# Plonky3/Plonky3-recursion

Measured on AMD Instinct MI355X. Metric: prove_next_layer ms + Poseidon2 perms/s, KoalaBear 2^20-row circuit, 1/8 GPU, lower is better.
Workload: dtype u32 Montgomery (31-bit prime field, degree-4 extension); Poseidon2 hashing as exact integers in f64; 1 GPU; prove_next_layer (verifier-circuit run on the device + prove_all_tables) of the synthetic koala-bear 2^20-row recursion layer: tables const/public/alu/poseidon2/recompose, FRI blowup 4, arity<=4, 54 queries, 15-bit PoW; circuit inputs + NextLayerPrepCache resident in HBM; field=koala-bear, log_height=20, independent_proofs=1, proof_bytes=612900, parallelism=1 independent proofs, one per GPU, no data-path collective

## Files before the change

plonky3_recursion_amd/csrc/kernels_coop.hip.h:

```cpp
#pragma once
#include "kernels.hip.h"

namespace p3r {

template <int CTRL>
__device__ __forceinline__ uint32_t dpp(uint32_t v) {
  return (uint32_t)__builtin_amdgcn_update_dpp(0, (int)v, CTRL, 0xF, 0xF, false);
}
constexpr int DPP_QUAD_NEXT1 = 0x39;
constexpr int DPP_QUAD_NEXT2 = 0x4E;
constexpr int DPP_QUAD_NEXT3 = 0x93;
constexpr int DPP_ROW_ROR1 = 0x121, DPP_ROW_ROR2 = 0x122, DPP_ROW_ROR4 = 0x124, DPP_ROW_ROR8 = 0x128;

template <class F>
__device__ __forceinline__ F coop_external(F x) {
  F b = F::raw(dpp<DPP_QUAD_NEXT1>(x.v)), c = F::raw(dpp<DPP_QUAD_NEXT2>(x.v)), d = F::raw(dpp<DPP_QUAD_NEXT3>(x.v));
  F ab = x + b;
  F y = ab.dbl() + b + (c + d);
  F t = y + F::raw(dpp<DPP_ROW_ROR4>(y.v));
  t = t + F::raw(dpp<DPP_ROW_ROR8>(t.v));
  return y + t;
}
template <class F>
__device__ __forceinline__ F coop_row_sum(F x) {
// ... 2 lines not shown
  t = t + F::raw(dpp<DPP_ROW_ROR2>(t.v));
  return t + F::raw(dpp<DPP_ROW_ROR1>(t.v));
}

constexpr int DPP_QUAD_BCAST0 = 0x00;
__device__ __forceinline__ uint32_t coop_bcast0(uint32_t x0) {
  uint32_t q = dpp<DPP_QUAD_BCAST0>(x0);
  q |= dpp<DPP_ROW_ROR4>(q);
  return q | dpp<DPP_ROW_ROR8>(q);
}

template <class PP>
struct CoopRc {
  uint32_t full[2 * P2_HALF_FULL];
  uint32_t part[PP::PARTIAL_ROUNDS];
};
template <class PP>
__device__ __forceinline__ CoopRc<PP> coop_load_rc(const uint32_t* __restrict__ rc, int elem) {
  CoopRc<PP> c;
#pragma unroll
  for (int r = 0; r < P2_HALF_FULL; ++r) c.full[r] = rc[r * P2_WIDTH + elem];
#pragma unroll
  for (int r = 0; r < PP::PARTIAL_ROUNDS; ++r) c.part[r] = rc[P2_HALF_FULL * P2_WIDTH + r];
#pragma unroll
  for (int r = 0; r < P2_HALF_FULL; ++r)
    c.full[P2_HALF_FULL + r] = rc[P2_HALF_FULL * P2_WIDTH + PP::PARTIAL_ROUNDS + r * P2_WIDTH + elem];
  return c;
}

template <class PP>
__device__ __forceinline__ Fp<PP> coop_permute(Fp<PP> s, int elem, Fp<PP> diag, const CoopRc<PP>& rc) {
  using F = Fp<PP>;
  s = coop_external(s);
#pragma unroll
  for (int r = 0; r < P2_HALF_FULL; ++r) {
    s = p2_sbox<PP>(s + F::raw(rc.full[r]));
    s = coop_external(s);
  }
#pragma unroll
  for (int r = 0; r < PP::PARTIAL_ROUNDS; ++r) {
    const F rest = coop_row_sum(elem == 0 ? F::zero() : s);
    const F sb = p2_sbox<PP>(s + F::raw(rc.part[r]));
    const F sum = rest + F::raw(coop_bcast0(elem == 0 ? sb.v : 0u));
    s = (elem == 0 ? sb : s) * diag + sum;
  }
#pragma unroll
  for (int r = 0; r < P2_HALF_FULL; ++r) {
    s = p2_sbox<PP>(s + F::raw(rc.full[P2_HALF_FULL + r]));
    s = coop_external(s);
  }
  return s;
}

template <class PP>
__global__ void __launch_bounds__(kBlock)
k_mmcs_hash_rows_strided_coop(const uint32_t* const* __restrict__ cols, int wtot, size_t h, size_t stride,
                              uint32_t* __restrict__ dig, const uint32_t* __restrict__ rc,
                              const uint32_t* __restrict__ diag) {
  using F = Fp<PP>;
  const size_t gid = (size_t)blockIdx.x * kBlock + threadIdx.x;
  const size_t row = gid >> 4;
  const int e = (int)(gid & 15);
  const bool live = row < h;
  const F d = F::raw(diag[e]);
  const CoopRc<PP> rcs = coop_load_rc<PP>(rc, e);
  F s = F::zero();
  for (int g = 0; g < wtot; g += P2_RATE) {
    if (live && e < P2_RATE && g + e < wtot) s = F::raw(cols[g + e][row * stride]);
    s = coop_permute<PP>(s, e, d, rcs);
  }
  if (live && e < P2_DIGEST) dig[(size_t)e * h + row] = s.v;
}

constexpr int kSubtreeBlock = 1024;
constexpr int kSubtreeNodes = 256;
constexpr int kSubtreeLevels = 8;
struct SubtreeArgs {
  const uint32_t* in;
  uint32_t n_in;
  uint32_t local;
  int n_levels;
  uint32_t* out[kSubtreeLevels];
  const uint32_t* inj[kSubtreeLevels];
  uint32_t* t_state;
  uint32_t* t_beta;
  uint32_t* t_cap;
  int t_dc;
};

template <class PP>
__device__ __forceinline__ void fri_transcript_step(int j, uint32_t root_word, uint32_t* __restrict__ state,
                                                    uint32_t* __restrict__ beta_out, uint32_t* __restrict__ cap_out,
                                                    const CoopRc<PP>& rc, const uint32_t* __restrict__ diag, int dc = 4) {
  using F = Fp<PP>;
  F s = j < P2_RATE ? F::raw(root_word) : F::raw(state[j]);
  if (j < P2_RATE) cap_out[j] = s.v;
  if (j == P2_RATE) s += F::from_canonical(P2_RATE);
  s = coop_permute<PP>(s, j, F::raw(diag[j]), rc);
  state[j] = s.v;
  if (j >= P2_RATE - dc && j < P2_RATE) beta_out[7 - j] = s.v;
}
template <class PP>
__global__ void __launch_bounds__(kSubtreeBlock)
k_mmcs_subtree(SubtreeArgs a, const uint32_t* __restrict__ rc, const uint32_t* __restrict__ diag) {
  using F = Fp<PP>;
  __shared__ uint32_t buf[2][P2_DIGEST * kSubtreeNodes / 2];
  const int elem = threadIdx.x & 15;
  const uint32_t group = threadIdx.x >> 4, k = elem & 7;
  const F d = F::raw(diag[elem]);
  const CoopRc<PP> rcs = coop_load_rc<PP>(rc, elem);
  uint32_t n = a.n_in < a.local ? a.n_in : a.local;
  uint32_t n_glob = a.n_in, first = blockIdx.x * n;
#pragma unroll
  for (int l = 0; l < kSubtreeLevels; ++l) {
    if (l < a.n_levels) {
      const uint32_t nn = n / 2, nn_glob = n_glob / 2, first_out = first / 2;
      const uint32_t* cur = buf[(l + 1) & 1];
      uint32_t* nxt = buf[l & 1];
      for (uint32_t node = group; node < nn; node += blockDim.x / 16) {
        const uint32_t child = 2 * node + (elem >> 3);
        F s = F::raw(l == 0 ? a.in[(size_t)k * n_glob + first + child] : cur[k * n + child]);
        s = coop_permute<PP>(s, elem, d, rcs);
        if (a.inj[l]) {
          if (elem >= P2_DIGEST) s = F::raw(a.inj[l][(size_t)k * nn_glob + first_out + node]);
          s = coop_permute<PP>(s, elem, d, rcs);
        }
        if (elem < P2_DIGEST) {
          nxt[k * nn + node] = s.v;
          a.out[l][(size_t)k * nn_glob + first_out + node] = s.v;
        }
      }
      __syncthreads();
      n = nn;
      n_glob = nn_glob;
      first = first_out;
    }
  }
  if (a.t_state && threadIdx.x < P2_WIDTH) {
    const uint32_t* root = buf[(a.n_levels - 1) & 1];
    fri_transcript_step<PP>((int)threadIdx.x, threadIdx.x < P2_RATE ? root[threadIdx.x] : 0u, a.t_state, a.t_beta,
                            a.t_cap, rcs, diag, a.t_dc ? a.t_dc : 4);
  }
}

template <class PP>
__global__ void __launch_bounds__(64)
k_fri_transcript_step(const uint32_t* __restrict__ root , uint32_t* __restrict__ state ,
                      uint32_t* __restrict__ beta_out , uint32_t* __restrict__ cap_out ,
                      const uint32_t* __restrict__ rc, const uint32_t* __restrict__ diag, int dc) {
  const int j = threadIdx.x;
  if (j >= P2_WIDTH) return;
  fri_transcript_step<PP>(j, j < P2_RATE ? root[j] : 0u, state, beta_out, cap_out, coop_load_rc<PP>(rc, j), diag, dc);
}



template <class F>
__device__ __forceinline__ F coop32_pair_sum(F t) {
  const auto r = __builtin_amdgcn_permlane16_swap(t.v, t.v, false, false);
  return F::raw(r[0]) + F::raw(r[1]);
}
template <class F>
__device__ __forceinline__ F coop32_external(F x) {
  const F b = F::raw(dpp<DPP_QUAD_NEXT1>(x.v)), c = F::raw(dpp<DPP_QUAD_NEXT2>(x.v)), d = F::raw(dpp<DPP_QUAD_NEXT3>(x.v));
  const F ab = x + b;
  const F y = ab.dbl() + b + (c + d);
  F t = y + F::raw(dpp<DPP_ROW_ROR4>(y.v));
  t = t + F::raw(dpp<DPP_ROW_ROR8>(t.v));
  return y + coop32_pair_sum(t);
}
template <class F>
__device__ __forceinline__ F coop32_sum(F x) { return coop32_pair_sum(coop_row_sum(x)); }
__device__ __forceinline__ uint32_t coop32_bcast0(uint32_t x0) {
  const uint32_t q = coop_bcast0(x0);
  const auto r = __builtin_amdgcn_permlane16_swap(q, q, false, false);
  return r[0] | r[1];
}

template <class PP>
// ... 45 lines not shown
```

plonky3_recursion_amd/csrc/kernels_stark.hip.h:

```cpp
#pragma once
#include "air_device.hip.h"
#include "kernels.hip.h"

namespace p3r {

template <int DC>
struct EW {
  uint32_t c[DC];
};
using E4 = EW<4>;
template <class PP, int DC = 4>
__host__ __device__ __forceinline__ typename Chal<PP, DC>::type e4_load(const EW<DC>& e) {
  typename Chal<PP, DC>::type r;
  for (int i = 0; i < DC; ++i) r.c[i] = Fp<PP>::raw(e.c[i]);
  return r;
}
template <class PP, int DC = 4>
__host__ __device__ __forceinline__ EW<DC> e4_store(const typename Chal<PP, DC>::type& e) {
  EW<DC> r;
  for (int i = 0; i < DC; ++i) r.c[i] = e.c[i].v;
  return r;
}

template <int DC>
// ... 350 lines not shown
#pragma unroll
    for (int i = 0; i < 4; ++i) out[i] = x[i].inv();
    return;
  }
  F t = p0123.inv();
  const F i3 = t * p012;
  t = t * nm[3].d;
  const F i2 = t * p01;
  t = t * nm[2].d;
  const F i1 = t * nm[0].d, i0 = t * nm[1].d;
  out[0] = x[0].inv_given(nm[0], i0);
  out[1] = x[1].inv_given(nm[1], i1);
  out[2] = x[2].inv_given(nm[2], i2);
  out[3] = x[3].inv_given(nm[3], i3);
}

}

#include "kernels_open.hip.h"

namespace p3r {

struct FriFoldArgs {
  const uint32_t* in;
  uint32_t* out;
  size_t rows;
  int log_rows;
  const uint32_t* beta;
  const uint32_t* roll;
  uint32_t w_inv;
  uint32_t tw_inv[4][8];
  uint32_t neg_half;
};
typedef uint32_t fri_u32x2 __attribute__((ext_vector_type(2)));
typedef uint32_t fri_u32x4 __attribute__((ext_vector_type(4)));
template <class PP, int DC, int LA, int S>
__device__ __forceinline__ void fri_fold_steps(typename Chal<PP, DC>::type* e, typename Chal<PP, DC>::type& b, Fp<PP>& ss_inv,
                                               const Fp<PP> nh, const uint32_t (&tw_inv)[4][8]) {
  using F = Fp<PP>;
  using E = typename Chal<PP, DC>::type;
  if constexpr (S < LA) {
#pragma unroll
    for (int j = 0; j < (1 << (LA - S - 1)); ++j) {
      F x0_inv = ss_inv * F::raw(tw_inv[S][j]);
      E t = b * x0_inv - E::one();
      e[j] = e[2 * j] + t * (e[2 * j + 1] - e[2 * j]) * nh;
    }
    ss_inv = ss_inv.sqr();
    b = b.sqr();
    fri_fold_steps<PP, DC, LA, S + 1>(e, b, ss_inv, nh, tw_inv);
  }
}
template <class PP, int DC, int LA>
__global__ void __launch_bounds__(kBlock) k_fri_fold(FriFoldArgs a) {
  using F = Fp<PP>;
  using E = typename Chal<PP, DC>::type;
  static_assert(LA >= 1 && LA <= 4, "folds by 2, 4, 8 or 16");
  constexpr int ARITY = 1 << LA;
  size_t r = (size_t)blockIdx.x * kBlock + threadIdx.x;
  if (r >= a.rows) return;
  const size_t n_in = a.rows << LA;
  E e[ARITY];
#pragma unroll
  for (int k = 0; k < DC; ++k) {
    const gptr<const uint32_t> row = as_global(a.in) + (size_t)k * n_in + (r << LA);
    if constexpr (LA == 1) {
      const fri_u32x2 v = *(gptr<const fri_u32x2>)row;
      e[0].c[k] = F::raw(v.x);
      e[1].c[k] = F::raw(v.y);
    } else {
#pragma unroll
      for (int q = 0; q < ARITY / 4; ++q) {
        const fri_u32x4 v = ((gptr<const fri_u32x4>)row)[q];
        e[4 * q].c[k] = F::raw(v.x);
        e[4 * q + 1].c[k] = F::raw(v.y);
        e[4 * q + 2].c[k] = F::raw(v.z);
        e[4 * q + 3].c[k] = F::raw(v.w);
      }
    }
  }
  F ss_inv = F::raw(a.w_inv).pow(bit_reverse((uint32_t)r, a.log_rows));
  E b;
#pragma unroll
  for (int k = 0; k < DC; ++k) b.c[k] = F::raw(as_global(a.beta)[k]);
  fri_fold_steps<PP, DC, LA, 0>(e, b, ss_inv, F::raw(a.neg_half), a.tw_inv);
  E res = e[0];
  if (a.roll) {
    E ro;
#pragma unroll
    for (int k = 0; k < DC; ++k) ro.c[k] = F::raw(as_global(a.roll)[(size_t)k * a.rows + r]);
    res += b * ro;
  }
#pragma unroll
  for (int k = 0; k < DC; ++k) as_global(a.out)[(size_t)k * a.rows + r] = res.c[k].v;
}

template <class PP>
__global__ void __launch_bounds__(kBlock)
k_mmcs_hash_rows_strided(const uint32_t* const* __restrict__ cols, int wtot, size_t h, size_t stride,
                         uint32_t* __restrict__ dig, const double* __restrict__ rcd) {
  size_t i = (size_t)blockIdx.x * kBlock + threadIdx.x;
  if (i >= h) return;
  double s[P2_WIDTH];
#pragma unroll
  for (int k = 0; k < P2_WIDTH; ++k) s[k] = 0.0;
  int g = 0;
  for (; g + P2_RATE <= wtot; g += P2_RATE) {
#pragma unroll
    for (int j = 0; j < P2_RATE; ++j) s[j] = p2f_load<PP>(cols[g + j][i * stride]);
    p2f_permute<PP, 0xFF00u>(s, rcd);
  }
  int rem = wtot - g;
  if (rem > 0) {
#pragma unroll
    for (int j = 0; j < P2_RATE; ++j)
      if (j < rem) s[j] = p2f_load<PP>(cols[g + j][i * stride]);
    p2f_permute<PP, 0xFFFFu>(s, rcd);
  }
#pragma unroll
  for (int k = 0; k < P2_DIGEST; ++k) dig[(size_t)k * h + i] = p2f_store<PP>(s[k]);
}

struct GrindArgs {
  uint32_t state[16];
  uint32_t pending[8];
  int n_pending;
  int bits;
  uint32_t base;
  const uint32_t* rc;
  uint32_t* result;
};
template <class PP>
__global__ void __launch_bounds__(kBlock) k_grind(GrindArgs a) {
  using F = Fp<PP>;
  uint32_t cand = a.base + blockIdx.x * kBlock + threadIdx.x;
  if (cand >= PP::P) return;
  F s[P2_WIDTH];
#pragma unroll
  for (int k = 0; k < P2_WIDTH; ++k) s[k] = F::raw(a.state[k]);
  const int n_abs = a.n_pending + 1;
#pragma unroll
  for (int k = 0; k < P2_RATE; ++k) {
    if (k < a.n_pending) s[k] = F::raw(a.pending[k]);
    else if (k == a.n_pending) s[k] = F::from_canonical(cand);
    else s[k] = F::zero();
  }
  s[P2_RATE] += F::from_canonical((uint32_t)n_abs);
// ... 29 lines not shown
```

plonky3_recursion_amd/csrc/mmcs_impl.hip.h:

```cpp

namespace {

template <class PP>
void hash_rows(p3r_ctx* ctx, const std::vector<std::vector<const p3r_dmat*>>& classes,
               const std::vector<uint32_t*>& digs) {
  std::vector<HashRowsJob> jobs;
  for (size_t c = 0; c < classes.size(); ++c) {
    std::vector<const uint32_t*> cols;
    for (const p3r_dmat* m : classes[c])
      for (size_t k = 0; k < m->w; ++k) cols.push_back(m->d + k * m->h);
    HashRowsJob j{};
    j.cols = col_table(ctx, cols);
    j.dig = digs[c];
    j.h = classes[c][0]->h;
    j.wtot = (int)cols.size();
    jobs.push_back(j);
  }
  std::stable_sort(jobs.begin(), jobs.end(),
                   [](const HashRowsJob& a, const HashRowsJob& b) { return a.wtot > b.wtot; });
  uint32_t blocks = 0;
  double perms = 0;
  for (auto& j : jobs) {
    j.block0 = blocks;
    blocks += blocks_for(j.h);
    perms += (double)j.h * ((j.wtot + P2_RATE - 1) / P2_RATE);
  }
  prof_count(ctx, "hash_rows_perms", perms);
  const auto* d_jobs =
      static_cast<const HashRowsJob*>(const_table(ctx, jobs.data(), jobs.size() * sizeof(HashRowsJob)));
  ProfScope ps(ctx, "mmcs_hash_rows");
  hipLaunchKernelGGL(k_mmcs_hash_rows<PP>, dim3(blocks), dim3(kBlock), 0, ctx->stream, d_jobs, (int)jobs.size(),
                     ctx->rcd());
  P3R_HIP(hipGetLastError());
}

inline size_t env_pow2(const char* name, size_t dflt, size_t lo, size_t hi) {
  const char* e = tuning_knob(name);
  size_t v = e ? (size_t)atol(e) : dflt;
  v = std::min(std::max(v, lo), hi);
  while (v & (v - 1)) v &= v - 1;
  return v;
}
inline size_t coop_max_nodes() {
  static const size_t v = env_pow2("P3R_COOP_MAX_NODES", 16384, 1, size_t(1) << 30);
  return v;
}
inline size_t coop_max_leaf_rows() {
  static const size_t v = env_pow2("P3R_COOP_MAX_LEAF_ROWS", 8192, 1, size_t(1) << 30);
  return v;
}
inline size_t subtree_nodes() {
  static const size_t v = env_pow2("P3R_SUBTREE_NODES", 32, 2, kSubtreeNodes);
  return v;
}
template <class PP>
void launch_compress(p3r_ctx* ctx, const uint32_t* prev, const uint32_t* inj, uint32_t* out, size_t n) {
  ProfScope ps(ctx, "mmcs_compress");
  hipLaunchKernelGGL(k_mmcs_compress<PP>, dim3(blocks_for(n)), dim3(kBlock), 0, ctx->stream, prev, inj, out, n,
                     ctx->rcd());
  P3R_HIP(hipGetLastError());
}

using InjectMap = std::map<size_t, DevBuf>;
inline const uint32_t* injected_at(const InjectMap* inject, const MmcsLevel& lv) {
  if (!lv.inject_h) return nullptr;
  if (!inject || !inject->count(lv.inject_h) || lv.inject_h != lv.logical_next)
    fail(P3R_EINVAL, "MMCS: matrix heights must be powers of two");
  return inject->at(lv.inject_h).p;
}
inline void push_layer(p3r_tree* tree, size_t n) {
  tree->layers.emplace_back(P2_DIGEST * n);
  tree->layer_n.push_back(n);
}

struct TranscriptStep {
  uint32_t *state, *beta, *cap;
  bool done = false;
  int dc = 4;
};
template <class PP>
size_t mmcs_subtree(p3r_ctx* ctx, p3r_tree* tree, size_t l, const InjectMap* inject, TranscriptStep* step) {
  const size_t n = tree->layer_n.back();
  if (n / 2 > coop_max_nodes()) return 0;
  SubtreeArgs a{};
  a.in = tree->layers.back().p;
  a.n_in = (uint32_t)n;
  const size_t local = std::min<size_t>(n, subtree_nodes());
  a.local = (uint32_t)local;
  for (size_t shrink = local; shrink > 1 && l + a.n_levels < tree->levels.size() && a.n_levels < kSubtreeLevels; shrink /= 2) {
    const MmcsLevel& lv = tree->levels[l + a.n_levels];
    push_layer(tree, lv.padded_next);
    a.out[a.n_levels] = tree->layers.back().p;
    a.inj[a.n_levels] = injected_at(inject, lv);
    ++a.n_levels;
  }
  if (step && tree->layer_n.back() == 1 && n == local) {
    a.t_state = step->state;
    a.t_beta = step->beta;
    a.t_cap = step->cap;
    a.t_dc = step->dc;
    step->done = true;
// ... 220 lines not shown
```

plonky3_recursion_amd/csrc/p3r_core.hip:

```cpp
#include "context.h"
#include "kernels.hip.h"
#include "kernels_stark.hip.h"
#include "kernels_coop.hip.h"
#include "tu_api.h"
#include "profile.h"
#include "run_schedule.h"
#include "prep_device.h"
#include "host_abi.h"

#include <sys/random.h>

#include <algorithm>
#include <cerrno>
#include <future>
#include <numeric>
#include <unordered_map>

using namespace p3r;

namespace {

thread_local std::string g_create_error;

template <class Fn>
int guard(p3r_ctx* ctx, Fn&& fn) {
  try {
    if (ctx) {
      (void)hipSetDevice(ctx->cfg.device);
      tls_pool() = ctx->pool;
      if (ctx->const_tables.size() > 4096) ctx->const_tables.clear();
    }
    fn();
    return P3R_OK;
  } catch (const Error& e) {
    if (ctx) ctx->err = e.what(); else g_create_error = e.what();
    return e.code;
  } catch (const std::exception& e) {
    if (ctx) ctx->err = e.what(); else g_create_error = e.what();
    return P3R_EINVAL;
  }
}

inline void require_w32_constants(const p3r_ctx* ctx) {
  if (ctx->w32_unacknowledged)
    fail(P3R_EINVAL, "the width-32 permutation with poseidon2_w32_rc / poseidon2_w32_diag NULL: the built-in constants are self-generated, "
                     "not upstream's - pass the caller's, or acknowledge with P3R_EXT_UNPINNED_W32_DEFAULTS");
}

#define P3R_FIELD_CALL(ctx, fn, ...)                                              \
  ((ctx)->cfg.field == P3R_FIELD_KOALA_BEAR ? fn<KoalaBearParams>(__VA_ARGS__)    \
                                            : fn<BabyBearParams>(__VA_ARGS__))

inline unsigned blocks_for(size_t n) { return (unsigned)((n + kBlock - 1) / kBlock); }

template <class PP>
std::unique_ptr<p3r_dmat> upload(p3r_ctx* ctx, const uint32_t* rowmajor, size_t h, size_t w) {
// ... 925 lines not shown
```

plonky3_recursion_amd/csrc/prove_impl.hip.h:

```cpp
#include "host_transcript.h"
#include "kernels_stark.hip.h"
#include "kernels_fri_reduce.hip.h"
#include "kernels_zk.hip.h"
#include "open_impl.hip.h"

struct p3r_prep {
  std::vector<p3r::AirParams> airs;
  std::vector<std::unique_ptr<p3r_dmat>> traces;
  std::vector<std::unique_ptr<p3r_dmat>> evals;
  std::vector<std::unique_ptr<p3r_dmat>> ldes;
  std::vector<size_t> heights;
  int zk_codewords = -1;
  const p3r_dmat* committed(size_t i) const { return evals.empty() ? traces[i].get() : evals[i].get(); }
  std::unique_ptr<p3r_tree> tree;
  std::vector<uint32_t> cap_canonical;
};

namespace {

template <class PP, int DC = 4>
EW<DC> to_e4(const typename Chal<PP, DC>::type& e) { return e4_store<PP, DC>(e); }

template <class PP, int DC = 4>
std::vector<typename Chal<PP, DC>::type> download_ef(p3r_ctx* ctx, const uint32_t* dev, size_t count) {
// ... 686 lines not shown
      FriReduceJob j{};
      j.ro = ros[kv.first].second.p;
      j.h = uint64_t(1) << kv.first;
      j.mat0 = (uint32_t)mats.size();
      j.n_mats = (uint32_t)kv.second.size();
      j.block0 = blocks;
      blocks += blocks_for(size_t(1) << kv.first);
      jobs.push_back(j);
      mats.insert(mats.end(), kv.second.begin(), kv.second.end());
    }
    const size_t b_mats = mats.size() * sizeof(FriReduceMatT<DC>), b_jobs = jobs.size() * sizeof(FriReduceJob),
                 b_vsum = vsum_jobs.size() * sizeof(FriVsumJob);
    const size_t o_jobs = (b_mats + 15) & ~size_t(15), o_vsum = (o_jobs + b_jobs + 15) & ~size_t(15);
    std::vector<unsigned char> blob(o_vsum + b_vsum);
    std::memcpy(blob.data(), mats.data(), b_mats);
    std::memcpy(blob.data() + o_jobs, jobs.data(), b_jobs);
    std::memcpy(blob.data() + o_vsum, vsum_jobs.data(), b_vsum);
    keep.emplace_back((blob.size() + 3) / 4);
    unsigned char* d_blob = reinterpret_cast<unsigned char*>(keep.back().p);
    P3R_HIP(ctx->stage.upload(ctx->stream, d_blob, blob.data(), blob.size()));
    const auto* d_mats = reinterpret_cast<const FriReduceMatT<DC>*>(d_blob);
    const auto* d_jobs = reinterpret_cast<const FriReduceJob*>(d_blob + o_jobs);
    const auto* d_vsum = reinterpret_cast<const FriVsumJob*>(d_blob + o_vsum);
    {
      ProfScope ps(ctx, "fri_reduce");
      hipLaunchKernelGGL((k_fri_vsum<PP, DC>), dim3((unsigned)vsum_jobs.size()), dim3(kBlock), 0, ctx->stream, d_vsum,
                         d_fapow.p);
      hipLaunchKernelGGL((k_fri_reduce_pre<PP, DC>), dim3(blocks), dim3(kBlock), 0, ctx->stream, d_jobs, (int)jobs.size(),
                         d_mats, d_fapow.p);
    }
    P3R_HIP(hipGetLastError());
  }

  void fri_commit_phase() {
    prof_stage(ctx, "fri_commit_phase");
    std::vector<int> heights;
    for (auto& kv : ros) heights.push_back(kv.first);
    std::sort(heights.rbegin(), heights.rend());
    log_max = heights[0];
    const int log_final = (int)cfg.log_final_poly_len + log_blowup;
    folded = std::move(ros[log_max].second);
    size_t next_h = 1;
    int log_cur = log_max;
    const bool device_transcript = cfg.cap_height == 0 && cfg.commit_pow_bits == 0 && ch.in_buf.empty();
    d_tstate.alloc(P2_WIDTH);
    d_phase.alloc((DC + P2_DIGEST) * kMaxPhases);
    uint32_t* const d_betas = d_phase.p;
    uint32_t* const d_caps = d_phase.p + DC * kMaxPhases;
    if (device_transcript) {
      uint32_t st[P2_WIDTH];
      for (int k = 0; k < P2_WIDTH; ++k) st[k] = ch.state[k].v;
      P3R_HIP(ctx->stage.upload(ctx->stream, d_tstate.p, st, sizeof st));
    }
    while (log_cur > log_final) {
      int log_next = next_h < heights.size() ? heights[next_h] : -1;
      int la = fri_log_arity(ctx->fri_log_arities, phases.size(), (int)cfg.max_log_arity, log_cur, log_final, log_next);
      if (la < 0) fail(P3R_EINVAL, "fri_log_arities does not fit the proof: phase %zu at height 2^%d", phases.size(), log_cur);
      if (la > 4) fail(P3R_EUNSUPPORTED, "max_log_arity > 4 is not supported");
      const size_t arity = size_t(1) << la, rows = (size_t(1) << log_cur) >> la;
      Phase ph{la, rows};
      commit_phase_leaves(ph, log_cur);
      const size_t pi = phases.size();
      if (pi >= kMaxPhases) fail(P3R_EUNSUPPORTED, "more than %zu FRI commit phases", kMaxPhases);
      TranscriptStep step{d_tstate.p, d_betas + DC * pi, d_caps + P2_DIGEST * pi};
      step.dc = DC;
      mmcs_build_levels<PP>(ctx, ph.tree.get(), nullptr, device_transcript ? &step : nullptr);
      if (device_transcript) {
        if (!step.done)
          hipLaunchKernelGGL(k_fri_transcript_step<PP>, dim3(1), dim3(64), 0, ctx->stream, ph.tree->layers.back().p,
                             step.state, step.beta, step.cap, ctx->rc.p, ctx->p2_diag.p, DC);
      } else {
        ph.cap = mmcs_cap_mont(ctx, ph.tree.get());
        for (uint32_t v : ph.cap) ch.observe(F::raw(v));
        commit_pow_witnesses.push_back(grind_witness<PP>(ctx, ch, (int)cfg.commit_pow_bits));
        const E beta = ch.sample_ext();
        uint32_t bw[DC];
        for (int k = 0; k < DC; ++k) bw[k] = beta.c[k].v;
        P3R_HIP(ctx->stage.upload(ctx->stream, d_betas + DC * pi, bw, sizeof bw));
      }
      DevBuf out(DC * rows);
      FriFoldArgs fa{};
      fa.in = folded.p; fa.out = out.p; fa.rows = rows; fa.log_rows = log_cur - la;
      fa.beta = d_betas + DC * pi;
      const bool roll = next_h < heights.size() && heights[next_h] == log_cur - la;
      fa.roll = roll ? ros[heights[next_h]].second.p : nullptr;
      fa.w_inv = F::two_adic_generator(log_cur).inv().v;
      const F omega = F::two_adic_generator(la);
      for (int s = 0; s < la; ++s) {
        F om_s = omega.pow(uint64_t(1) << s);
        for (int j = 0; j < (int)(arity >> (s + 1)); ++j)
          fa.tw_inv[s][j] = om_s.pow(bit_reverse(2 * j, la - s)).inv().v;
      }
      fa.neg_half = (-(F::from_canonical(2).inv())).v;
      {
        ProfScope ps(ctx, "fri_fold");
        static constexpr void (*kFold[4])(FriFoldArgs) = {k_fri_fold<PP, DC, 1>, k_fri_fold<PP, DC, 2>, k_fri_fold<PP, DC, 3>,
                                                          k_fri_fold<PP, DC, 4>};
        hipLaunchKernelGGL(kFold[la - 1], dim3(blocks_for(rows)), dim3(kBlock), 0, ctx->stream, fa);
      }
      P3R_HIP(hipGetLastError());
      if (roll) ++next_h;
      ph.folded_in = std::move(folded);
      folded = std::move(out);
      log_cur -= la;
      phases.push_back(std::move(ph));
    }
    if (next_h != heights.size()) fail(P3R_EINVAL, "FRI: an input height was never rolled in");
    final_polynomial(log_cur, device_transcript);
    for (auto& c : final_poly) ch.observe_ext(c);
    for (auto& ph : phases) ch.observe(F::from_canonical((uint32_t)ph.la));
    query_pow_witness = grind_witness<PP>(ctx, ch, (int)cfg.query_pow_bits);
  }

  void commit_phase_leaves(Phase& ph, int log_cur) {
    const size_t arity = size_t(1) << ph.la, rows = ph.rows, n_in = size_t(1) << log_cur;
    if ((int)cfg.cap_height > log_cur - ph.la)
      fail(P3R_EINVAL, "cap_height %d exceeds the height of FRI commit phase %zu (2^%d rows)", (int)cfg.cap_height,
           phases.size(), log_cur - ph.la);
    ph.tree = std::make_unique<p3r_tree>();
    mmcs_begin(ctx, ph.tree.get(), {rows});
    std::vector<const uint32_t*> cols;
    for (size_t j = 0; j < arity; ++j)
      for (int k = 0; k < DC; ++k) cols.push_back(folded.p + (size_t)k * n_in + j);
    if (cfg.mmcs_salt_elems) {
      const uint32_t S = cfg.mmcs_salt_elems;
      p3r_tree& T = *ph.tree;
      T.salt_elems = (int)S; T.phase_salt_stride = arity; T.phase_rows = rows;
      T.phase_salts.alloc((size_t)S * n_in);
      std::vector<ZkTileJob> tj(1);
      tj[0].dst = T.phase_salts.p; tj[0].rows = rows; tj[0].w2 = S; tj[0].mode = 1; tj[0].stride = (uint32_t)arity;
      tj[0].stream = zk_stream_id(kSaltRoundFri, phases.size());
      launch_zk_tiles<PP>(ctx, tj, zk_key, "mmcs_salts");
      for (uint32_t c = 0; c < S; ++c) cols.push_back(T.phase_salts.p + (size_t)c * n_in);
    }
    mmcs_hash_rows_strided<PP>(ctx, ph.tree.get(), cols, rows, arity);
  }

  void final_polynomial(int log_cur, bool device_transcript) {
    const size_t m = size_t(1) << log_cur;
    std::vector<uint32_t> raw(DC * m), phase_words(d_phase.n);
    if (device_transcript && !phases.empty()) P3R_HIP(fetch_small(ctx, d_phase.p, phase_words.size(), phase_words.data()));
    P3R_HIP(fetch_small(ctx, folded.p, raw.size(), raw.data()));
    const uint32_t* betas = phase_words.data();
    const uint32_t* caps = betas + DC * kMaxPhases;
    if (device_transcript) {
      for (size_t pi = 0; pi < phases.size(); ++pi) {
        phases[pi].cap.assign(caps + P2_DIGEST * pi, caps + P2_DIGEST * (pi + 1));
        for (uint32_t v : phases[pi].cap) ch.observe(F::raw(v));
        commit_pow_witnesses.push_back(grind_witness<PP>(ctx, ch, 0));
        const E beta = ch.sample_ext();
        for (int k = 0; k < DC; ++k)
          if (beta.c[k].v != betas[DC * pi + k]) fail(P3R_EHIP, "internal: device and host FRI transcripts disagree");
      }
    }
    std::vector<E> coeffs(m);
    for (size_t i = 0; i < m; ++i)
      for (int k = 0; k < DC; ++k) coeffs[i].c[k] = F::raw(raw[(size_t)k * m + i]);
    const F w_inv = F::two_adic_generator(log_cur).inv(), m_inv = F::from_u64(m).inv();
    for (size_t len = 2; len <= m; len <<= 1) {
      const F w_len = w_inv.pow(m / len);
// ... 253 lines not shown
```

plonky3_recursion_amd/device.py:

```python
import ctypes as C

import numpy as np

from . import _lib

FIELD_IDS = {"koala-bear": _lib.FIELD_KOALA_BEAR, "baby-bear": _lib.FIELD_BABY_BEAR}
MODULUS = {"koala-bear": 0x7F000001, "baby-bear": 0x78000001}
GENERATOR = {"koala-bear": 3, "baby-bear": 31}


class P3rError(RuntimeError):
    def __init__(self, code, msg):
        super().__init__(f"p3r error {code}: {msg}")
        self.code = code


def _u32(a):
    a = np.ascontiguousarray(a, dtype=np.uint32)
    return a, a.ctypes.data_as(_lib.u32p)


def _u8(a):
    a = np.ascontiguousarray(a, dtype=np.uint8)
    return a, a.ctypes.data_as(C.POINTER(C.c_uint8))
# ... 338 lines not shown

    def prep_create(self, airs, prep_mats):
        n = len(airs)
        descs = (_lib.P3rAirDesc * n)()
        arr = (_lib.P3rMatrix * n)()
        keep = []
        for i, (a, m) in enumerate(zip(airs, prep_mats)):
            descs[i].kind = a["kind"]
            descs[i].lanes = a.get("lanes", 1)
            descs[i].horner_packed_steps = a.get("horner_packed_steps", 2)
            descs[i].coeff_lookups = a.get("coeff_lookups", 0)
            x, p = _u32(m)
            keep.append(x)
            arr[i].values, arr[i].height, arr[i].width = p, x.shape[0], x.shape[1]
        cap = np.empty((1 << self.cap_height, 8), dtype=np.uint32)
        h = self.ptr(self.lib.p3r_prep_create(self.h, descs, arr, n, cap.ctypes.data_as(_lib.u32p)))
        return cap, ProverData(self, h)

    def _proof_call(self, fn, *args):
        buf = getattr(self, "_proof_buf", None)
        if buf is None:
            buf = self._proof_buf = C.create_string_buffer(1 << 20)
        n = C.c_size_t()
        rc = fn(*args, C.cast(buf, C.POINTER(C.c_uint8)), len(buf), C.byref(n))
        if rc == -6 and n.value > len(buf):
            buf = self._proof_buf = C.create_string_buffer(max(n.value + n.value // 4, 2 * len(buf)))
            rc = self.lib.p3r_take_proof(self.h, C.cast(buf, C.POINTER(C.c_uint8)), len(buf), C.byref(n))
        self.check(rc)
        return C.string_at(buf, n.value)

    def prove_batch(self, prover_data, main_traces, canonical_field_encoding=False):
        flags = 1 if canonical_field_encoding else 0
        n = len(main_traces)
        if all(isinstance(m, DeviceMatrix) for m in main_traces):
            arr = (C.c_void_p * n)(*[m.h for m in main_traces])
            return self._proof_call(self.lib.p3r_prove_batch, self.h, prover_data.h, arr, n, flags)
        arr = (_lib.P3rMatrix * n)()
        keep = []
        for i, m in enumerate(main_traces):
            x, p = _u32(m)
            keep.append(x)
            arr[i].values, arr[i].height, arr[i].width = p, x.shape[0], x.shape[1]
        return self._proof_call(self.lib.p3r_prove_batch_host, self.h, prover_data.h, arr, n, flags)

    def profile_enable(self, on=True):
        self.check(self.lib.p3r_profile_enable(self.h, 1 if on else 0))

    def trim(self):
        n = C.c_uint64()
        self.check(self.lib.p3r_trim(self.h, C.byref(n)))
        return n.value

    def profile_read(self):
        buf = (_lib.P3rProfileEntry * 64)()
        n = C.c_size_t()
        self.check(self.lib.p3r_profile_read(self.h, buf, 64, C.byref(n)))
        return {buf[i].name.decode(): (buf[i].total_ms, buf[i].launches) for i in range(n.value)}

    def time_permute(self, dmat, iters):
        ms = C.c_double()
        self.check(self.lib.p3r_time_permute_dmat(self.h, dmat.h, iters, C.byref(ms)))
        return ms.value


class DeviceMatrix:
    def __init__(self, ctx, handle):
        self.ctx, self.h = ctx, handle

    @property
    def shape(self):
        return (self.ctx.lib.p3r_dmat_height(self.h), self.ctx.lib.p3r_dmat_width(self.h))

    def download(self):
        out = np.empty(self.shape, dtype=np.uint32)
        self.ctx.check(self.ctx.lib.p3r_dmat_download(self.ctx.h, self.h, out.ctypes.data_as(_lib.u32p)))
        return out

    def free(self):
        if self.h and self.ctx.h:
            self.ctx.lib.p3r_dmat_free(self.ctx.h, self.h)
        self.h = None

    def __del__(self):
        try:
            self.free()
        except Exception:
            pass


class ProverData:

    def __init__(self, ctx, handle):
        self.ctx, self.h = ctx, handle

    def free(self):
        if self.h and self.ctx.h:
            self.ctx.lib.p3r_prep_free(self.ctx.h, self.h)
        self.h = None

    def __del__(self):
        try:
            self.free()
        except Exception:
            pass


class DeviceP2Rows:
    def __init__(self, ctx, handle):
        self.ctx, self.h = ctx, handle
# ... 62 lines not shown
```

Measured before the change: 25.33 ms.

## Fuse small FRI commit-phase rounds into one single-block tail kernel

Once the FRI layer height drops below a threshold (2^8 by default), every remaining commit round runs inside one 1024-thread block of a single kernel. Each round does leaf hashing, Merkle levels, the transcript permutation and the fold. This replaces several small kernel launches per round (leaf hash, subtree, transcript step, fold) with one launch driven by a device-side round table. It removes launch latency on tiny workloads. The cost is running everything in one block with __syncthreads between stages, and a gate that only applies without zk, salt or arity-4 MMCS.

```diff
diff --git a/plonky3_recursion_amd/csrc/kernels_coop.hip.h b/plonky3_recursion_amd/csrc/kernels_coop.hip.h
--- a/plonky3_recursion_amd/csrc/kernels_coop.hip.h
+++ b/plonky3_recursion_amd/csrc/kernels_coop.hip.h
@@ -78,6 +78,17 @@
   return s;
 }
 
+template <class PP, class Load>
+__device__ __forceinline__ Fp<PP> coop_sponge_row(int e, int wtot, bool live, Fp<PP> d, const CoopRc<PP>& rcs, Load load) {
+  using F = Fp<PP>;
+  F s = F::zero();
+  for (int g = 0; g < wtot; g += P2_RATE) {
+    if (live && e < P2_RATE && g + e < wtot) s = F::raw(load(g + e));
+    s = coop_permute<PP>(s, e, d, rcs);
+  }
+  return s;
+}
+
 template <class PP>
 __global__ void __launch_bounds__(kBlock)
 k_mmcs_hash_rows_strided_coop(const uint32_t* const* __restrict__ cols, int wtot, size_t h, size_t stride,
@@ -88,13 +99,8 @@
   const size_t row = gid >> 4;
   const int e = (int)(gid & 15);
   const bool live = row < h;
-  const F d = F::raw(diag[e]);
-  const CoopRc<PP> rcs = coop_load_rc<PP>(rc, e);
-  F s = F::zero();
-  for (int g = 0; g < wtot; g += P2_RATE) {
-    if (live && e < P2_RATE && g + e < wtot) s = F::raw(cols[g + e][row * stride]);
-    s = coop_permute<PP>(s, e, d, rcs);
-  }
+  const F s = coop_sponge_row<PP>(e, wtot, live, F::raw(diag[e]), coop_load_rc<PP>(rc, e),
+                                  [&](int c) { return cols[c][row * stride]; });
   if (live && e < P2_DIGEST) dig[(size_t)e * h + row] = s.v;
 }
 
@@ -115,7 +121,7 @@
 };
 
 template <class PP>
-__device__ __forceinline__ void fri_transcript_step(int j, uint32_t root_word, uint32_t* __restrict__ state,
+__device__ __forceinline__ Fp<PP> fri_transcript_step(int j, uint32_t root_word, uint32_t* __restrict__ state,
                                                     uint32_t* __restrict__ beta_out, uint32_t* __restrict__ cap_out,
                                                     const CoopRc<PP>& rc, const uint32_t* __restrict__ diag, int dc = 4) {
   using F = Fp<PP>;
@@ -125,6 +131,17 @@
   s = coop_permute<PP>(s, j, F::raw(diag[j]), rc);
   state[j] = s.v;
   if (j >= P2_RATE - dc && j < P2_RATE) beta_out[7 - j] = s.v;
+  return s;
+}
+template <class PP>
+__device__ __forceinline__ Fp<PP> subtree_node(uint32_t own, const uint32_t* inj, int elem, Fp<PP> d, const CoopRc<PP>& rcs) {
+  using F = Fp<PP>;
+  F s = coop_permute<PP>(F::raw(own), elem, d, rcs);
+  if (inj) {
+    if (elem >= P2_DIGEST) s = F::raw(*inj);
+    s = coop_permute<PP>(s, elem, d, rcs);
+  }
+  return s;
 }
 template <class PP>
 __global__ void __launch_bounds__(kSubtreeBlock)
@@ -145,12 +162,8 @@
       uint32_t* nxt = buf[l & 1];
       for (uint32_t node = group; node < nn; node += blockDim.x / 16) {
         const uint32_t child = 2 * node + (elem >> 3);
-        F s = F::raw(l == 0 ? a.in[(size_t)k * n_glob + first + child] : cur[k * n + child]);
-        s = coop_permute<PP>(s, elem, d, rcs);
-        if (a.inj[l]) {
-          if (elem >= P2_DIGEST) s = F::raw(a.inj[l][(size_t)k * nn_glob + first_out + node]);
-          s = coop_permute<PP>(s, elem, d, rcs);
-        }
+        const uint32_t own = l == 0 ? a.in[(size_t)k * n_glob + first + child] : cur[k * n + child];
+        const F s = subtree_node<PP>(own, a.inj[l] ? a.inj[l] + (size_t)k * nn_glob + first_out + node : nullptr, elem, d, rcs);
         if (elem < P2_DIGEST) {
           nxt[k * nn + node] = s.v;
           a.out[l][(size_t)k * nn_glob + first_out + node] = s.v;
diff --git a/plonky3_recursion_amd/csrc/kernels_fri_tail.hip.h b/plonky3_recursion_amd/csrc/kernels_fri_tail.hip.h
--- /dev/null
+++ b/plonky3_recursion_amd/csrc/kernels_fri_tail.hip.h
@@ -0,0 +1,86 @@
+#pragma once
+#include "kernels_coop.hip.h"
+#include "kernels_stark.hip.h"
+
+namespace p3r {
+
+constexpr int kFriTailBlock = 1024;
+constexpr int kFriTailMaxLog = 12;
+constexpr int kFriTailDefaultLog = 8;
+struct FriTailRound {
+  FriFoldArgs fold;
+  int la;
+  int n_levels;
+  uint32_t* cap;
+  uint32_t* layers[kFriTailMaxLog];
+};
+
+template <class PP, int DC, int LA>
+__device__ __forceinline__ void fri_tail_fold(const FriFoldArgs& fa, const uint32_t* s_beta) {
+  typename Chal<PP, DC>::type b;
+#pragma unroll
+  for (int k = 0; k < DC; ++k) b.c[k] = Fp<PP>::raw(s_beta[k]);
+  for (size_t r = threadIdx.x; r < fa.rows; r += kFriTailBlock) fri_fold_row<PP, DC, LA>(fa, b, r);
+}
+
+template <class PP, int DC>
+__global__ void __launch_bounds__(kFriTailBlock)
+k_fri_commit_tail(const FriTailRound* __restrict__ rounds, int n_rounds, uint32_t* __restrict__ t_state,
+                  const uint32_t* __restrict__ rc, const uint32_t* __restrict__ diag) {
+  using F = Fp<PP>;
+  __shared__ uint32_t s_beta[8];
+  if (blockIdx.x != 0) return;
+  const int elem = threadIdx.x & 15;
+  const uint32_t group = threadIdx.x >> 4, k = elem & 7;
+  constexpr uint32_t kGroups = kFriTailBlock / 16;
+  for (int rd = 0; rd < n_rounds; ++rd) {
+    const uint32_t* rc_r = rc;
+    const uint32_t* diag_r = diag;
+    asm volatile("" : "+s"(rc_r), "+s"(diag_r));
+    const F d = F::raw(diag_r[elem]);
+    const CoopRc<PP> rcs = coop_load_rc<PP>(rc_r, elem);
+    const FriTailRound& R = rounds[rd];
+    const FriFoldArgs& fa = R.fold;
+    const int la = R.la;
+    const uint32_t rows = (uint32_t)fa.rows, n_in = rows << la;
+    {
+      const gptr<const uint32_t> in = as_global(fa.in);
+      const gptr<uint32_t> dig = as_global(R.layers[0]);
+      for (uint32_t row = group; row < rows; row += kGroups) {
+        const F s = coop_sponge_row<PP>(elem, DC << la, true, d, rcs, [&](int c) {
+          return in[(size_t)(c % DC) * n_in + ((size_t)row << la) + (uint32_t)(c / DC)];
+        });
+        if (elem < P2_DIGEST) dig[(size_t)elem * rows + row] = s.v;
+      }
+    }
+    __syncthreads();
+    uint32_t n = rows;
+    for (int l = 0; l < R.n_levels; ++l) {
+      const uint32_t nn = n / 2;
+      const gptr<const uint32_t> cur = as_global(R.layers[l]);
+      const gptr<uint32_t> nxt = as_global(R.layers[l + 1]);
+      for (uint32_t node = group; node < nn; node += kGroups) {
+        const F s = subtree_node<PP>(cur[(size_t)k * n + 2 * node + (elem >> 3)], nullptr, elem, d, rcs);
+        if (elem < P2_DIGEST) nxt[(size_t)k * nn + node] = s.v;
+      }
+      __syncthreads();
+      n = nn;
+    }
+    if (threadIdx.x < P2_WIDTH) {
+      const int j = (int)threadIdx.x;
+      const uint32_t root_word = j < P2_RATE ? as_global(R.layers[R.n_levels])[j] : 0u;
+      const F s = fri_transcript_step<PP>(j, root_word, t_state, const_cast<uint32_t*>(fa.beta), R.cap, rcs, diag_r, DC);
+      if (j >= P2_RATE - DC && j < P2_RATE) s_beta[7 - j] = s.v;
+    }
+    __syncthreads();
+    switch (la) {
+      case 1: fri_tail_fold<PP, DC, 1>(fa, s_beta); break;
+      case 2: fri_tail_fold<PP, DC, 2>(fa, s_beta); break;
+      case 3: fri_tail_fold<PP, DC, 3>(fa, s_beta); break;
+      default: fri_tail_fold<PP, DC, 4>(fa, s_beta); break;
+    }
+    __syncthreads();
+  }
+}
+
+}
diff --git a/plonky3_recursion_amd/csrc/kernels_stark.hip.h b/plonky3_recursion_amd/csrc/kernels_stark.hip.h
--- a/plonky3_recursion_amd/csrc/kernels_stark.hip.h
+++ b/plonky3_recursion_amd/csrc/kernels_stark.hip.h
@@ -426,13 +426,11 @@
   }
 }
 template <class PP, int DC, int LA>
-__global__ void __launch_bounds__(kBlock) k_fri_fold(FriFoldArgs a) {
+__device__ __forceinline__ void fri_fold_row(const FriFoldArgs& a, typename Chal<PP, DC>::type b, size_t r) {
   using F = Fp<PP>;
   using E = typename Chal<PP, DC>::type;
   static_assert(LA >= 1 && LA <= 4, "folds by 2, 4, 8 or 16");
   constexpr int ARITY = 1 << LA;
-  size_t r = (size_t)blockIdx.x * kBlock + threadIdx.x;
-  if (r >= a.rows) return;
   const size_t n_in = a.rows << LA;
   E e[ARITY];
 #pragma unroll
@@ -454,9 +452,6 @@
     }
   }
   F ss_inv = F::raw(a.w_inv).pow(bit_reverse((uint32_t)r, a.log_rows));
-  E b;
-#pragma unroll
-  for (int k = 0; k < DC; ++k) b.c[k] = F::raw(as_global(a.beta)[k]);
   fri_fold_steps<PP, DC, LA, 0>(e, b, ss_inv, F::raw(a.neg_half), a.tw_inv);
   E res = e[0];
   if (a.roll) {
@@ -467,6 +462,16 @@
   }
 #pragma unroll
   for (int k = 0; k < DC; ++k) as_global(a.out)[(size_t)k * a.rows + r] = res.c[k].v;
+}
+template <class PP, int DC, int LA>
+__global__ void __launch_bounds__(kBlock) k_fri_fold(FriFoldArgs a) {
+  using F = Fp<PP>;
+  const size_t r = (size_t)blockIdx.x * kBlock + threadIdx.x;
+  if (r >= a.rows) return;
+  typename Chal<PP, DC>::type b;
+#pragma unroll
+  for (int k = 0; k < DC; ++k) b.c[k] = F::raw(as_global(a.beta)[k]);
+  fri_fold_row<PP, DC, LA>(a, b, r);
 }
 
 template <class PP>
diff --git a/plonky3_recursion_amd/csrc/mmcs_impl.hip.h b/plonky3_recursion_amd/csrc/mmcs_impl.hip.h
--- a/plonky3_recursion_amd/csrc/mmcs_impl.hip.h
+++ b/plonky3_recursion_amd/csrc/mmcs_impl.hip.h
@@ -47,6 +47,13 @@
 }
 inline size_t coop_max_leaf_rows() {
   static const size_t v = env_pow2("P3R_COOP_MAX_LEAF_ROWS", 8192, 1, size_t(1) << 30);
+  return v;
+}
+inline int fri_tail_max_log() {
+  static const int v = [] {
+    const char* e = tuning_knob("P3R_FRI_TAIL_MAX_LOG");
+    return e ? std::min(std::max(atoi(e), 0), kFriTailMaxLog) : kFriTailDefaultLog;
+  }();
   return v;
 }
 inline size_t subtree_nodes() {
diff --git a/plonky3_recursion_amd/csrc/p3r_core.hip b/plonky3_recursion_amd/csrc/p3r_core.hip
--- a/plonky3_recursion_amd/csrc/p3r_core.hip
+++ b/plonky3_recursion_amd/csrc/p3r_core.hip
@@ -2,6 +2,7 @@
 #include "kernels.hip.h"
 #include "kernels_stark.hip.h"
 #include "kernels_coop.hip.h"
+#include "kernels_fri_tail.hip.h"
 #include "tu_api.h"
 #include "profile.h"
 #include "run_schedule.h"
diff --git a/plonky3_recursion_amd/csrc/prove_impl.hip.h b/plonky3_recursion_amd/csrc/prove_impl.hip.h
--- a/plonky3_recursion_amd/csrc/prove_impl.hip.h
+++ b/plonky3_recursion_amd/csrc/prove_impl.hip.h
@@ -762,12 +762,67 @@
       for (int k = 0; k < P2_WIDTH; ++k) st[k] = ch.state[k].v;
       P3R_HIP(ctx->stage.upload(ctx->stream, d_tstate.p, st, sizeof st));
     }
+    auto next_la = [&](int cur, size_t nh) {
+      const int log_next = nh < heights.size() ? heights[nh] : -1;
+      const int la = fri_log_arity(ctx->fri_log_arities, phases.size(), (int)cfg.max_log_arity, cur, log_final, log_next);
+      if (la < 0) fail(P3R_EINVAL, "fri_log_arities does not fit the proof: phase %zu at height 2^%d", phases.size(), cur);
+      if (la > 4) fail(P3R_EUNSUPPORTED, "max_log_arity > 4 is not supported");
+      return la;
+    };
+    auto fold_args = [&](int cur, int la, size_t nh, size_t pi, const uint32_t* in, uint32_t* out, bool* roll) {
+      FriFoldArgs fa{};
+      fa.in = in; fa.out = out; fa.rows = (size_t(1) << cur) >> la; fa.log_rows = cur - la;
+      fa.beta = d_betas + DC * pi;
+      *roll = nh < heights.size() && heights[nh] == cur - la;
+      fa.roll = *roll ? ros[heights[nh]].second.p : nullptr;
+      fa.w_inv = F::two_adic_generator(cur).inv().v;
+      const F omega = F::two_adic_generator(la);
+      for (int s = 0; s < la; ++s) {
+        F om_s = omega.pow(uint64_t(1) << s);
+        for (int j = 0; j < (1 << la >> (s + 1)); ++j)
+          fa.tw_inv[s][j] = om_s.pow(bit_reverse(2 * j, la - s)).inv().v;
+      }
+      fa.neg_half = (-(F::from_canonical(2).inv())).v;
+      return fa;
+    };
+    const bool tail_ok = device_transcript && cfg.mmcs_arity != 4 && cfg.mmcs_salt_elems == 0 && !zk;
+    const size_t launches0 = ctx->prof.size();
     while (log_cur > log_final) {
-      int log_next = next_h < heights.size() ? heights[next_h] : -1;
-      int la = fri_log_arity(ctx->fri_log_arities, phases.size(), (int)cfg.max_log_arity, log_cur, log_final, log_next);
-      if (la < 0) fail(P3R_EINVAL, "fri_log_arities does not fit the proof: phase %zu at height 2^%d", phases.size(), log_cur);
-      if (la > 4) fail(P3R_EUNSUPPORTED, "max_log_arity > 4 is not supported");
-      const size_t arity = size_t(1) << la, rows = (size_t(1) << log_cur) >> la;
+      if (tail_ok && log_cur <= fri_tail_max_log()) {
+        std::vector<FriTailRound> tab;
+        while (log_cur > log_final) {
+          const int la = next_la(log_cur, next_h);
+          const size_t rows = (size_t(1) << log_cur) >> la, pi = phases.size();
+          if (pi >= kMaxPhases) fail(P3R_EUNSUPPORTED, "more than %zu FRI commit phases", kMaxPhases);
+          Phase ph{la, rows};
+          ph.tree = std::make_unique<p3r_tree>();
+          mmcs_begin(ctx, ph.tree.get(), {rows});
+          for (const MmcsLevel& lv : ph.tree->levels) push_layer(ph.tree.get(), lv.padded_next);
+          DevBuf out(DC * rows);
+          bool roll = false;
+          FriTailRound R{};
+          R.fold = fold_args(log_cur, la, next_h, pi, folded.p, out.p, &roll);
+          R.la = la;
+          R.n_levels = (int)ph.tree->levels.size();
+          R.cap = d_caps + P2_DIGEST * pi;
+          if (R.n_levels >= kFriTailMaxLog) fail(P3R_EHIP, "internal: FRI tail round of %zu rows", rows);
+          for (size_t l = 0; l < ph.tree->layers.size(); ++l) R.layers[l] = ph.tree->layers[l].p;
+          tab.push_back(R);
+          if (roll) ++next_h;
+          ph.folded_in = std::move(folded);
+          folded = std::move(out);
+          log_cur -= la;
+          phases.push_back(std::move(ph));
+        }
+        const auto* d_tab = static_cast<const FriTailRound*>(const_table(ctx, tab.data(), tab.size() * sizeof(FriTailRound)));
+        ProfScope ps(ctx, "fri_commit_tail");
+        hipLaunchKernelGGL((k_fri_commit_tail<PP, DC>), dim3(1), dim3(kFriTailBlock), 0, ctx->stream, d_tab, (int)tab.size(),
+                           d_tstate.p, ctx->rc.p, ctx->p2_diag.p);
+        P3R_HIP(hipGetLastError());
+        break;
+      }
+      const int la = next_la(log_cur, next_h);
+      const size_t rows = (size_t(1) << log_cur) >> la;
       Phase ph{la, rows};
       commit_phase_leaves(ph, log_cur);
       const size_t pi = phases.size();
@@ -776,9 +831,11 @@
       step.dc = DC;
       mmcs_build_levels<PP>(ctx, ph.tree.get(), nullptr, device_transcript ? &step : nullptr);
       if (device_transcript) {
-        if (!step.done)
+        if (!step.done) {
+          ProfScope ps(ctx, "fri_transcript_step");
           hipLaunchKernelGGL(k_fri_transcript_step<PP>, dim3(1), dim3(64), 0, ctx->stream, ph.tree->layers.back().p,
                              step.state, step.beta, step.cap, ctx->rc.p, ctx->p2_diag.p, DC);
+        }
       } else {
         ph.cap = mmcs_cap_mont(ctx, ph.tree.get());
         for (uint32_t v : ph.cap) ch.observe(F::raw(v));
@@ -789,19 +846,8 @@
         P3R_HIP(ctx->stage.upload(ctx->stream, d_betas + DC * pi, bw, sizeof bw));
       }
       DevBuf out(DC * rows);
-      FriFoldArgs fa{};
-      fa.in = folded.p; fa.out = out.p; fa.rows = rows; fa.log_rows = log_cur - la;
-      fa.beta = d_betas + DC * pi;
-      const bool roll = next_h < heights.size() && heights[next_h] == log_cur - la;
-      fa.roll = roll ? ros[heights[next_h]].second.p : nullptr;
-      fa.w_inv = F::two_adic_generator(log_cur).inv().v;
-      const F omega = F::two_adic_generator(la);
-      for (int s = 0; s < la; ++s) {
-        F om_s = omega.pow(uint64_t(1) << s);
-        for (int j = 0; j < (int)(arity >> (s + 1)); ++j)
-          fa.tw_inv[s][j] = om_s.pow(bit_reverse(2 * j, la - s)).inv().v;
-      }
-      fa.neg_half = (-(F::from_canonical(2).inv())).v;
+      bool roll = false;
+      const FriFoldArgs fa = fold_args(log_cur, la, next_h, pi, folded.p, out.p, &roll);
       {
         ProfScope ps(ctx, "fri_fold");
         static constexpr void (*kFold[4])(FriFoldArgs) = {k_fri_fold<PP, DC, 1>, k_fri_fold<PP, DC, 2>, k_fri_fold<PP, DC, 3>,
@@ -816,6 +862,7 @@
       phases.push_back(std::move(ph));
     }
     if (next_h != heights.size()) fail(P3R_EINVAL, "FRI: an input height was never rolled in");
+    prof_count(ctx, "fri_commit_launches", (double)(ctx->prof.size() - launches0));
     final_polynomial(log_cur, device_transcript);
     for (auto& c : final_poly) ch.observe_ext(c);
     for (auto& ph : phases) ch.observe(F::from_canonical((uint32_t)ph.la));
diff --git a/plonky3_recursion_amd/device.py b/plonky3_recursion_amd/device.py
--- a/plonky3_recursion_amd/device.py
+++ b/plonky3_recursion_amd/device.py
@@ -414,9 +414,9 @@
         return n.value
 
     def profile_read(self):
-        buf = (_lib.P3rProfileEntry * 64)()
+        buf = (_lib.P3rProfileEntry * 128)()
         n = C.c_size_t()
-        self.check(self.lib.p3r_profile_read(self.h, buf, 64, C.byref(n)))
+        self.check(self.lib.p3r_profile_read(self.h, buf, 128, C.byref(n)))
         return {buf[i].name.decode(): (buf[i].total_ms, buf[i].launches) for i in range(n.value)}
 
     def time_permute(self, dmat, iters):
```

Measured after the change: 25.65 ms. 1.3% more time.
